# lighttransport/pbrlab

Measured on AMD Instinct MI355X. Metric: Msamples/s (paths x spp / s), 1920x1080 Cornell-box-Suzanne render, higher is better.
Workload: dtype f32

## Files before the change

pbrlab_amd/csrc/bvh_build.cpp:

```cpp
#include <math.h>
#include <stdlib.h>
#include <string.h>

#include <algorithm>
#include <atomic>
#include <deque>
#include <functional>
#include <future>
#include <limits>
#include <thread>

#include "host_scene.h"

namespace pb {
namespace {

#ifndef PB_SAH_BINS
#define PB_SAH_BINS 48
#endif
constexpr int kBins = PB_SAH_BINS;
#ifndef PB_SAH_SWEEP
#define PB_SAH_SWEEP 256
#endif
#ifndef PB_MAX_LEAF_CURVES
// ... 210 lines not shown
    work.push_back({root, 0});
    while (!work.empty()) {
      Item it;
      if (N.size() < (size_t)kTopNodes) it = work.front(), work.pop_front();
      else it = work.back(), work.pop_back();
      const TNode& t = T[it.t];
      depth = std::max(depth, t.depth);
      BvhNode nd;
      memset(&nd, 0, sizeof(nd));
      const TNode &l = T[t.left], &r = T[t.right];
      nd.set_box(0, l.box.lo, l.box.hi);
      nd.set_box(1, r.box.lo, r.box.hi);
      if (l.left < 0) {
        nd.c0 = leaf_ref(l);
      } else {
        nd.c0 = (uint32_t)N.size();
        N.emplace_back();
        work.push_back({t.left, nd.c0});
      }
      if (r.left < 0) {
        nd.c1 = leaf_ref(r);
      } else {
        nd.c1 = (uint32_t)N.size();
        N.emplace_back();
        work.push_back({t.right, nd.c1});
      }
      N[it.out] = nd;
    }
  }
  out->slot_gid = b.order;
  out->depth = depth;
}

struct QBox {
  float lo[3], hi[3];
};
static bool quantise_node(const QBox* c, int n, QNode* nd) {
  memset(nd, 0, sizeof(*nd));
  uint32_t* qw[6] = {&nd->qlo_x, &nd->qlo_y, &nd->qlo_z, &nd->qhi_x, &nd->qhi_y, &nd->qhi_z};
  for (int a = 0; a < 3; a++) {
    float lo = std::numeric_limits<float>::infinity(), hi = -lo;
    for (int i = 0; i < n; i++) lo = std::min(lo, c[i].lo[a]), hi = std::max(hi, c[i].hi[a]);
    if (!(lo <= hi) || !std::isfinite(lo) || !std::isfinite(hi)) return false;
    float sc = std::max(nextafterf((hi - lo) / 253.0f, std::numeric_limits<float>::infinity()), 1.1754944e-38f);
    for (int tries = 0;; tries++) {
      if (tries > 40 || !std::isfinite(sc)) return false;
      const float org = lo;
      bool ok = true;
      uint32_t wl = 0, wh = 0;
      for (int i = 0; i < 4 && ok; i++) {
        if (i >= n) {
          wl |= 255u << (8 * i);
          continue;
        }
        int ql = (int)floor(((double)c[i].lo[a] - (double)org) / (double)sc);
        int qh = (int)ceil(((double)c[i].hi[a] - (double)org) / (double)sc);
        ql = std::max(0, std::min(255, ql)), qh = std::max(0, std::min(255, qh));
        while (ql > 0 && !(fmaf((float)ql, sc, org) <= c[i].lo[a])) ql--;
        while (qh < 255 && !(fmaf((float)qh, sc, org) >= c[i].hi[a])) qh++;
        if (!(fmaf((float)ql, sc, org) <= c[i].lo[a] && fmaf((float)qh, sc, org) >= c[i].hi[a])) ok = false;
        wl |= (uint32_t)ql << (8 * i), wh |= (uint32_t)qh << (8 * i);
      }
      if (ok) {
        nd->org[a] = org;
        (a == 0 ? nd->sx : (a == 1 ? nd->sy : nd->sz)) = sc;
        *qw[a] = wl, *qw[3 + a] = wh;
        break;
      }
      sc *= tries < 8 ? 1.03125f : 2.0f;
    }
  }
  return true;
}

uint32_t build_qtree(const std::vector<BvhNode>& N2, const std::function<uint32_t(uint32_t)>& map_leaf, std::vector<QNode>* out) {
  out->clear();
  if (N2.empty()) return 0;
  struct V {
    float lo[3], hi[3];
    int32_t l = -1, r = -1;
    uint32_t ref = 0;
    uint32_t prims = 0;
  };
  std::vector<V> T;
  T.reserve(N2.size() * 2 + 1);
  {
    struct Todo {
      uint32_t node2;
      int32_t v;
    };
    std::vector<Todo> todo;
    T.emplace_back();
    todo.push_back({0u, 0});
    while (!todo.empty()) {
      const Todo t = todo.back();
      todo.pop_back();
      const BvhNode& b = N2[t.node2];
      int32_t kids[2] = {-1, -1};
      int nk = 0;
      for (int k = 0; k < 2; k++) {
        const uint32_t ref = k ? b.c1 : b.c0;
        if (ref == kEmptyChild) continue;
        const int32_t v = (int32_t)T.size();
        T.emplace_back();
        for (int a = 0; a < 3; a++) T[v].lo[a] = b.lo[a][k], T[v].hi[a] = b.hi[a][k];
        kids[nk++] = v;
        if (ref & kLeafBit) T[v].ref = map_leaf(ref), T[v].prims = (ref & 7u) + 1u;
        else todo.push_back({ref, v});
      }
      if (nk == 2) T[t.v].l = kids[0], T[t.v].r = kids[1];
      else if (nk == 1) T[t.v].l = kids[0], T[t.v].r = -1;
    }
    for (int a = 0; a < 3; a++) {
      T[0].lo[a] = std::numeric_limits<float>::infinity(), T[0].hi[a] = -T[0].lo[a];
      for (int32_t k : {T[0].l, T[0].r})
        if (k >= 0) T[0].lo[a] = std::min(T[0].lo[a], T[k].lo[a]), T[0].hi[a] = std::max(T[0].hi[a], T[k].hi[a]);
    }
  }
  auto area = [](const V& v) {
    const float dx = v.hi[0] - v.lo[0], dy = v.hi[1] - v.lo[1], dz = v.hi[2] - v.lo[2];
    const float a = dx * dy + dy * dz + dz * dx;
    return a >= 0.f && std::isfinite(a) ? (double)a : 0.0;
  };
  constexpr double kCostNode = 1.0, kCostPrim = 1.0;
  const size_t nv = T.size();
  std::vector<double> below(nv, 0.0);
  std::vector<int32_t> choice(nv * 4, -1);
  auto qarea = [&](const V& u, const V& v) {
    double e[3];
    for (int a = 0; a < 3; a++) {
      const double ext = (double)v.hi[a] - (double)v.lo[a];
      const double st = std::max(ext / 253.0, 1e-37);
      const double ql = floor(((double)u.lo[a] - (double)v.lo[a]) / st), qh = ceil(((double)u.hi[a] - (double)v.lo[a]) / st);
      e[a] = std::max(qh - ql, 0.0) * st;
    }
    const double a = e[0] * e[1] + e[1] * e[2] + e[2] * e[0];
    return std::isfinite(a) ? a : 0.0;
  };
  for (size_t vi = nv; vi-- > 0;) {
    const V& v = T[vi];
    if (v.l < 0) continue;
    if (v.r < 0) {
      choice[vi * 4] = v.l;
      below[vi] = T[v.l].l < 0 ? area(T[v.l]) * kCostPrim * T[v.l].prims : area(T[v.l]) * kCostNode + below[v.l];
      continue;
    }
    int32_t fronts[16][4];
    int sizes[16], nf = 0;
    fronts[0][0] = v.l, fronts[0][1] = v.r, sizes[0] = 2, nf = 1;
    for (int i = 0; i < nf && nf < 16; i++) {
      if (sizes[i] >= 4) continue;
      for (int m = 0; m < sizes[i] && nf < 16; m++) {
        const V& u = T[fronts[i][m]];
        if (u.l < 0 || u.r < 0) continue;
        int32_t g[4];
        int n = 0;
        for (int j = 0; j < sizes[i]; j++) {
          if (j == m) g[n++] = u.l, g[n++] = u.r;
          else g[n++] = fronts[i][j];
        }
        std::sort(g, g + n);
        bool dup = false;
        for (int q = 0; q < nf && !dup; q++) dup = sizes[q] == n && std::equal(g, g + n, fronts[q]);
        if (dup) continue;
        std::copy(g, g + n, fronts[nf]), sizes[nf] = n, nf++;
// ... 1 lines not shown
    }
    double best = 1e300;
    int bi = 0;
    for (int i = 0; i < nf; i++) {
      double c = 0.0;
      for (int m = 0; m < sizes[i]; m++) {
        const V& u = T[fronts[i][m]];
        c += u.l < 0 ? qarea(u, v) * kCostPrim * u.prims : qarea(u, v) * kCostNode + below[fronts[i][m]];
      }
      if (c < best) best = c, bi = i;
    }
    below[vi] = best;
    for (int m = 0; m < sizes[bi]; m++) choice[vi * 4 + m] = fronts[bi][m];
  }
  struct Item {
    int32_t v;
    uint32_t out;
  };
  std::deque<Item> work;
  out->emplace_back();
  work.push_back({0, 0u});
  while (!work.empty()) {
    Item it;
    if (out->size() < (size_t)kTopNodes) it = work.front(), work.pop_front();
    else it = work.back(), work.pop_back();
    int32_t fr[4];
    int n = 0;
    if (T[it.v].l < 0) {
      fr[n++] = it.v;
    } else {
      for (int m = 0; m < 4; m++)
        if (choice[(size_t)it.v * 4 + m] >= 0) fr[n++] = choice[(size_t)it.v * 4 + m];
    }
    QBox c[4];
    for (int i = 0; i < n; i++)
      for (int a = 0; a < 3; a++) c[i].lo[a] = T[fr[i]].lo[a], c[i].hi[a] = T[fr[i]].hi[a];
    QNode nd;
    if (n == 0 || !quantise_node(c, n, &nd)) {
      out->clear();
      return 0;
    }
    for (int i = 0; i < 4; i++) nd.c[i] = kEmptyChild;
    for (int i = 0; i < n; i++) {
      const V& u = T[fr[i]];
      if (u.l < 0) {
        nd.c[i] = u.ref;
      } else {
        const uint32_t id = (uint32_t)out->size();
        out->emplace_back();
        nd.c[i] = id;
        work.push_back({fr[i], id});
      }
    }
    (*out)[it.out] = nd;
  }
  std::vector<uint32_t> need(out->size(), 0);
  for (size_t i = out->size(); i-- > 0;) {
    const QNode& nd = (*out)[i];
    uint32_t nc = 0, deepest = 0;
    for (int k = 0; k < 4; k++) {
      if (nd.c[k] == kEmptyChild) continue;
      nc++;
      if (!(nd.c[k] & kLeafBit)) deepest = std::max(deepest, need[nd.c[k]]);
    }
    need[i] = (nc ? nc - 1u : 0u) + deepest;
  }
  return need[0];
}

void build_qlayout(const FlatBvh& bvh, const std::vector<float4>& slots, const std::vector<uint8_t>& kinds, QLayout* out) {
  static_assert(kMaxLeaf <= 2, "a leaf of the binary tree becomes one TriPair / one curve record");
  *out = QLayout();
  std::vector<float4>&qtri = out->tri, &qpts = out->pts;
  std::vector<uint32_t>& qhit = out->hit;
  const float4 zero = make_float4(0.f, 0.f, 0.f, 0.f);
  auto code = [&](uint32_t k) { return k | __builtin_bit_cast(uint32_t, slots[4 * (size_t)k + 2].w); };
  const bool tri_pairs = std::all_of(kinds.begin(), kinds.end(), [](uint8_t kd) { return kd == 0; });
  auto tri_leaf = [&](uint32_t first, uint32_t count) -> uint32_t {
    if (!tri_pairs) {
      const uint32_t rec = (uint32_t)(qtri.size() / 3);
      for (uint32_t i = 0; i < count; i++) {
        for (int c = 0; c < 3; c++) qtri.push_back(slots[4 * (size_t)(first + i) + c]);
        qtri.back().w = __builtin_bit_cast(float, code(first + i));
      }
      return rec;
    }
    const uint32_t rec = (uint32_t)(qtri.size() / kTriPairWords);
    const float4* a = &slots[4 * (size_t)first];
    const float4* b = count == 2 ? &slots[4 * (size_t)(first + 1)] : a;
    const float ca = __builtin_bit_cast(float, code(first)), cb = __builtin_bit_cast(float, count == 2 ? code(first + 1) : kNone);
    qtri.insert(qtri.end(), {make_float4(a[0].x, b[0].x, a[0].y, b[0].y), make_float4(a[0].z, b[0].z, a[1].x, b[1].x),
                             make_float4(a[1].y, b[1].y, a[1].z, b[1].z), make_float4(a[2].x, b[2].x, a[2].y, b[2].y),
                             make_float4(a[2].z, b[2].z, ca, cb)});
    return rec;
  };
  qpts.assign(4, zero);
  qhit.assign(4, kNone);
  auto curve_leaf = [&](uint32_t first, uint32_t count) -> uint32_t {
    while (qpts.size() % 4) qpts.push_back(zero);
    const uint32_t P = (uint32_t)qpts.size();
    uint32_t sub[2] = {0u, 0u};
    for (uint32_t i = 0; i < count; i++) {
      const float4* sl = &slots[4 * (size_t)(first + i)];
      qpts.push_back(sl[0]), qpts.push_back(sl[1]);
      sub[i] = __builtin_bit_cast(uint32_t, sl[2].x) & 3u;
    }
    qhit.resize(qpts.size(), kNone);
    qhit[P] = code(first);
    if (count == 2) qhit[P + 2] = code(first + 1);
    (count == 2 ? out->leaves_pair : out->leaves_one)++;
    return kLeafBit | kCurveBit | ((P | sub[0]) << 3) | (count == 2 ? (kCurvePairBit | sub[1]) : 0u);
  };
  auto map_leaf = [&](uint32_t ref) -> uint32_t {
    const uint32_t first = (ref & 0x3FFFFFFFu) >> 3, count = (ref & 7u) + 1u;
    if (ref & kCurveBit) return curve_leaf(first, count);
    return kLeafBit | (tri_leaf(first, count) << 3) | (count - 1u);
  };
  out->stack_need = build_qtree(bvh.nodes, map_leaf, &out->nodes);
  if (out->stack_need > (uint32_t)kStackDepth || qpts.size() >= (1u << 27)) out->nodes.clear();
  while (qtri.size() % 4) qtri.push_back(zero);
  for (int k = 0; k < 4; k++) qpts.push_back(zero);
  qhit.resize(qpts.size(), kNone);
}

std::vector<SssEntry> build_sss_entries(const std::vector<QNode>& wide, const std::vector<float>& ilo, const std::vector<float>& ihi,
                                        uint32_t max_foreign) {
  const size_t ninst = ilo.size() / 3;
  std::vector<SssEntry> entries(ninst, SssEntry{});
  struct CutRef { uint32_t ref; float lo[3], hi[3]; };
  for (size_t i = 0; i < ninst; i++) {
    SssEntry& E = entries[i];
    if (!(ilo[3 * i] <= ihi[3 * i])) continue;
    float ext = 0.f;
    for (int a = 0; a < 3; a++) ext = std::max(ext, ihi[3 * i + a] - ilo[3 * i + a]);
    if (!(ext > 0.f) || !std::isfinite(ext)) continue;
    const float m1 = 1e-4f * ext, m2 = 2e-3f * ext;
    float rlo[3], rhi[3], wlo[3], whi[3];
    for (int a = 0; a < 3; a++) rlo[a] = ilo[3 * i + a] - m1, rhi[a] = ihi[3 * i + a] + m1, wlo[a] = rlo[a] - m2, whi[a] = rhi[a] + m2;
    std::vector<CutRef> cut{{0u, {-INFINITY, -INFINITY, -INFINITY}, {INFINITY, INFINITY, INFINITY}}};
    for (bool changed = true; changed;) {
      changed = false;
      for (size_t c = 0; c < cut.size() && !changed; c++) {
        if (cut[c].ref & kLeafBit) continue;
        const QNode& nd = wide[cut[c].ref];
        const float org[3] = {nd.org[0], nd.org[1], nd.org[2]}, st3[3] = {nd.sx, nd.sy, nd.sz};
        const uint32_t ql[3] = {nd.qlo_x, nd.qlo_y, nd.qlo_z}, qh[3] = {nd.qhi_x, nd.qhi_y, nd.qhi_z};
        std::vector<CutRef> kids;
        int nchild = 0;
        for (int k = 0; k < 4; k++) {
          if (nd.c[k] == kEmptyChild) continue;
          nchild++;
          CutRef r;
          r.ref = nd.c[k];
          bool meets = true;
          for (int a = 0; a < 3; a++) {
            r.lo[a] = fmaf((float)((ql[a] >> (8 * k)) & 255u), st3[a], org[a]);
            r.hi[a] = fmaf((float)((qh[a] >> (8 * k)) & 255u), st3[a], org[a]);
            meets = meets && r.lo[a] <= whi[a] && r.hi[a] >= wlo[a];
          }
          if (meets) kids.push_back(r);
        }
        if (((int)kids.size() < nchild || kids.size() == 1) && cut.size() - 1 + kids.size() <= 1u + max_foreign) {
          cut.erase(cut.begin() + (ptrdiff_t)c);
          cut.insert(cut.end(), kids.begin(), kids.end());
          changed = true;
        }
      }
    }
    int best = -1;
    double best_v = -1.0;
    for (size_t c = 0; c < cut.size(); c++) {
      if (cut[c].ref & kLeafBit) continue;
      double v = 1.0;
      for (int a = 0; a < 3; a++) v *= std::max(0.0, (double)std::min(cut[c].hi[a], ihi[3 * i + a]) - (double)std::max(cut[c].lo[a], ilo[3 * i + a]));
      if (v > best_v) best_v = v, best = (int)c;
    }
    if (best < 0 || cut[(size_t)best].ref == 0u) continue;
    E.entry = cut[(size_t)best].ref;
// ... 13 lines not shown
```

pbrlab_amd/csrc/dscene.h:

```cpp
#pragma once
#include <math.h>

#include "dclosures.h"

namespace pb {

constexpr uint32_t kLeafBit = 0x80000000u;
constexpr uint32_t kCurveBit = 0x40000000u;
constexpr uint32_t kEmptyChild = 0xFFFFFFFFu;
#ifndef PB_MAX_LEAF
#define PB_MAX_LEAF 2
#endif
constexpr int kMaxLeaf = PB_MAX_LEAF;
#ifndef PB_STACK_DEPTH
#define PB_STACK_DEPTH 64
#endif
constexpr int kStackDepth = PB_STACK_DEPTH;
constexpr int kSimpleLdsStack = 40;
#ifndef PB_TOP_NODES
#define PB_TOP_NODES 64
#endif
constexpr int kTopNodes = PB_TOP_NODES;
#ifndef PB_TOP_NODES_WIDE
#define PB_TOP_NODES_WIDE 0
#endif
constexpr int kTopNodesWide = PB_TOP_NODES_WIDE;

struct alignas(16) BvhNode {
  float lo[3][2];
  float hi[3][2];
  uint32_t c0, c1;
  uint32_t pad[2];
  static float widen_lo(float v) { return v - (fabsf(v) * 1.52587890625e-05f + 1e-30f); }
  static float widen_hi(float v) { return v + (fabsf(v) * 1.52587890625e-05f + 1e-30f); }
  void set_box(int child, const float* l, const float* h) {
    for (int a = 0; a < 3; a++) lo[a][child] = widen_lo(l[a]), hi[a][child] = widen_hi(h[a]);
  }
};
static_assert(sizeof(BvhNode) == 64, "node must be 64 B");

constexpr uint32_t kCurvePairBit = 4u;
struct alignas(16) QNode {
  float org[3], sx;
  float sy, sz;
  uint32_t qlo_x, qlo_y;
  uint32_t qlo_z, qhi_x, qhi_y, qhi_z;
  uint32_t c[4];
};
static_assert(sizeof(QNode) == 64, "quantised wide node must be 64 B");
constexpr uint32_t kTriPairWords = 5;

constexpr uint32_t kQPointHit = 0x80000000u;

constexpr uint32_t kSlotHasNormals = 1u;
constexpr uint32_t kSlotIsCurve = 2u;
constexpr uint32_t kSlotMatHair = 4u;
constexpr uint32_t kSlotMatNone = 8u;
constexpr uint32_t kSlotHasUV = 16u;

struct alignas(128) ShadeRec {
  float ng[3];
  uint32_t matflags;
  float ns_flat[3];
  uint32_t lightrec;
  float n[9];
  uint32_t pad0;
  float uv[6];
  uint32_t gid, instance_id, geom_id, prim_id;
  uint32_t pad[4];
};
static_assert(sizeof(ShadeRec) == 128, "one cache line per primitive");

constexpr uint32_t kHitSlotMask = 0x07FFFFFFu;
constexpr uint32_t kHitMore = 1u << 27;
constexpr uint32_t kHitHair = 1u << 28;
constexpr uint32_t kHitLight = 1u << 29;
constexpr uint32_t kHitNoMaterial = 1u << 30;

struct PrincipledBsdf {
  int enable_diffuse;
// ... 128 lines not shown
```

pbrlab_amd/csrc/dtrace.h:

```cpp
#pragma once

#include "dscene.h"

namespace pb {

struct Hit {
  float t, u, v;
  uint32_t slot;
};

struct TravStats {
  uint32_t nodes, tris, curves;
  uint32_t anodes, atris, acurves;
  uint32_t it_node, it_tri, it_curve, it_refill, ln_node, ln_tri, ln_curve;
  uint32_t hist[8], max_steps;
  uint32_t ahist[8], amax_steps;
  uint32_t refill_ticks;
  unsigned long long cyc[4];
  uint32_t suspended, suspended_any;
  unsigned long long t_exhausted;
};

__device__ __forceinline__ V3 ld3(const float4& a) { return V3(a.x, a.y, a.z); }

// ... 174 lines not shown
  float dist = (ey * pxa - ex * pya) / sqrtf(len2);
  float r = a.w + s * (b.w - a.w);
  if (!(r > 0.0f && fabsf(dist) <= r)) return false;
  float tt = (pza + s * (pzb - pza)) * inv_len;
  if (!(tt > tmin && tt <= tmax)) return false;
  const float rm = __builtin_fmaxf(fabsf(a.w), fabsf(b.w));
  const V3 lo(__builtin_fminf(a.x, b.x) - rm, __builtin_fminf(a.y, b.y) - rm, __builtin_fminf(a.z, b.z) - rm);
  const V3 hi(__builtin_fmaxf(a.x, b.x) + rm, __builtin_fmaxf(a.y, b.y) + rm, __builtin_fmaxf(a.z, b.z) + rm);
  if (!hit_inside(lo, hi, o, inv3, tt)) return false;
  t = tt, u = ((float)i + s) * 0.25f, v = dist / r;
  return true;
}

__device__ __forceinline__ void box_test2(const float4& n0, const float4& n1, const float4& n2, V3 o, V3 inv, float tmin,
                                          float tmax, bool& h0, bool& h1, float& t0, float& t1) {
  const f2 ox = {o.x, o.x}, oy = {o.y, o.y}, oz = {o.z, o.z};
  const f2 ix = {inv.x, inv.x}, iy = {inv.y, inv.y}, iz = {inv.z, inv.z};
  const f2 lx = {n0.x, n0.y}, ly = {n0.z, n0.w}, lz = {n1.x, n1.y};
  const f2 hx = {n1.z, n1.w}, hy = {n2.x, n2.y}, hz = {n2.z, n2.w};
  f2 p = (lx - ox) * ix, q = (hx - ox) * ix;
  f2 a = __builtin_elementwise_min(p, q), b = __builtin_elementwise_max(p, q);
  p = (ly - oy) * iy, q = (hy - oy) * iy;
  a = __builtin_elementwise_max(a, __builtin_elementwise_min(p, q)), b = __builtin_elementwise_min(b, __builtin_elementwise_max(p, q));
  p = (lz - oz) * iz, q = (hz - oz) * iz;
  a = __builtin_elementwise_max(a, __builtin_elementwise_min(p, q)), b = __builtin_elementwise_min(b, __builtin_elementwise_max(p, q));
  const float e = 1.52587890625e-05f;
  const float a0 = __builtin_fmaf(-fabsf(a.x), e, a.x), a1 = __builtin_fmaf(-fabsf(a.y), e, a.y);
  const float b0 = __builtin_fmaf(fabsf(b.x), e, b.x), b1 = __builtin_fmaf(fabsf(b.y), e, b.y);
  t0 = a0, t1 = a1;
  h0 = a0 <= b0 && b0 >= tmin && a0 <= tmax;
  h1 = a1 <= b1 && b1 >= tmin && a1 <= tmax;
}

__device__ __forceinline__ void box_test4q(const float4& w0, const float4& w1, const float4& w2, V3 o, const float4& inv, float ta[4],
                                           float tb[4]) {
  const float e = 1.52587890625e-05f;
  const bool nx = (int)__float_as_uint(inv.x) < 0, ny = (int)__float_as_uint(inv.y) < 0, nz = (int)__float_as_uint(inv.z) < 0;
  const uint32_t qlx = __float_as_uint(w1.z), qly = __float_as_uint(w1.w), qlz = __float_as_uint(w2.x);
  const uint32_t qhx = __float_as_uint(w2.y), qhy = __float_as_uint(w2.z), qhz = __float_as_uint(w2.w);
  const uint32_t lx = nx ? qhx : qlx, ly = ny ? qhy : qly, lz = nz ? qhz : qlz;
  const uint32_t hx = nx ? qlx : qhx, hy = ny ? qly : qhy, hz = nz ? qlz : qhz;
  const f2 sx = {w0.w, w0.w}, sy = {w1.x, w1.x}, sz = {w1.y, w1.y}, gx = {w0.x, w0.x}, gy = {w0.y, w0.y}, gz = {w0.z, w0.z};
  const f2 ox = {o.x, o.x}, oy = {o.y, o.y}, oz = {o.z, o.z}, ix = {inv.x, inv.x}, iy = {inv.y, inv.y}, iz = {inv.z, inv.z};
#pragma unroll
  for (int h = 0; h < 2; h++) {
    auto two = [h](uint32_t w) { return h ? f2{(float)((w >> 16) & 255u), (float)(w >> 24)} : f2{(float)(w & 255u), (float)((w >> 8) & 255u)}; };
    const f2 px = (__builtin_elementwise_fma(two(lx), sx, gx) - ox) * ix, qx = (__builtin_elementwise_fma(two(hx), sx, gx) - ox) * ix;
    const f2 py = (__builtin_elementwise_fma(two(ly), sy, gy) - oy) * iy, qy = (__builtin_elementwise_fma(two(hy), sy, gy) - oy) * iy;
    const f2 pz = (__builtin_elementwise_fma(two(lz), sz, gz) - oz) * iz, qz = (__builtin_elementwise_fma(two(hz), sz, gz) - oz) * iz;
    const float a0 = __builtin_fmaxf(__builtin_fmaxf(px.x, py.x), pz.x), a1 = __builtin_fmaxf(__builtin_fmaxf(px.y, py.y), pz.y);
    const float b0 = __builtin_fminf(__builtin_fminf(qx.x, qy.x), qz.x), b1 = __builtin_fminf(__builtin_fminf(qx.y, qy.y), qz.y);
    ta[2 * h] = __builtin_fmaf(-fabsf(a0), e, a0), ta[2 * h + 1] = __builtin_fmaf(-fabsf(a1), e, a1);
    tb[2 * h] = __builtin_fmaf(fabsf(b0), e, b0), tb[2 * h + 1] = __builtin_fmaf(fabsf(b1), e, b1);
  }
}

constexpr uint32_t kWideMiss = 0xFFFFFFFFu;
__device__ __forceinline__ void wide_node_keys(const float4& w0, const float4& w1, const float4& w2, const float4& refs, V3 o,
                                               const float4& inv, float tmin, float tmax, uint32_t k[4]) {
  float ta[4], tb[4];
  box_test4q(w0, w1, w2, o, inv, ta, tb);
  const uint32_t r[4] = {__float_as_uint(refs.x), __float_as_uint(refs.y), __float_as_uint(refs.z), __float_as_uint(refs.w)};
#pragma unroll
  for (int i = 0; i < 4; i++) {
    const bool h = ta[i] <= tb[i] && tb[i] >= tmin && ta[i] <= tmax && r[i] != kEmptyChild;
    const int bits = (int)__float_as_uint(ta[i]);
    k[i] = h ? ((uint32_t)(bits < 0 ? 0 : bits) & ~3u) | (uint32_t)i : kWideMiss;
  }
  auto cex = [](uint32_t& a, uint32_t& b) {
    const uint32_t lo = a < b ? a : b, hi = a < b ? b : a;
    a = lo, b = hi;
  };
  cex(k[0], k[1]), cex(k[2], k[3]), cex(k[0], k[2]), cex(k[1], k[3]), cex(k[1], k[2]);
}
__device__ __forceinline__ uint32_t wide_ref(const float4& refs, uint32_t key) {
  const uint32_t a = __float_as_uint((key & 1u) ? refs.y : refs.x), b = __float_as_uint((key & 1u) ? refs.w : refs.z);
  return (key & 2u) ? b : a;
}

__device__ __forceinline__ uint32_t q_gid(const DScene& sc, uint32_t code) {
  const uint32_t c = (code & kQPointHit) ? sc.q_hitcode[code & ~kQPointHit] : code;
  return sc.shade[c & kHitSlotMask].gid;
}
__device__ __forceinline__ uint32_t q_final_code(const DScene& sc, uint32_t code) {
  return (code != kNone && (code & kQPointHit)) ? sc.q_hitcode[code & ~kQPointHit] : code;
}

template <int MODE, bool STATS, bool CURVES, bool WIDE = false>
__device__ __forceinline__ bool leaf_test(const DScene& sc, uint32_t leaf, V3 o, V3 d, V3 inv, float tmin, float& best_t,
                                          Hit& hit, TravStats& st, bool any_rt) {
  const bool ANY = MODE == 2 ? any_rt : (MODE == 1);
  uint32_t first = (leaf & 0x3FFFFFFFu) >> 3, count = (leaf & 7u) + 1u;
  bool is_curve = (leaf & kCurveBit) != 0;
  if (WIDE && !CURVES) {
    const float4* g = sc.wide + sc.q_tri0 + (size_t)first * kTriPairWords;
    const float4 w0 = g[0], w1 = g[1], w2 = g[2], w3 = g[3], w4 = g[4];
    uint32_t nt = 0u;
    const bool occluded = tri_pair_accept<MODE == 1, STATS>(sc, w0, w1, w2, w3, w4, o, d, inv, tmin, ANY, hit, nt);
    if (STATS) st.tris += nt;
    best_t = hit.t;
    return occluded;
  }
  const bool rec = WIDE && CURVES && is_curve;
  const uint32_t sub_a = first & 3u, sub_b = leaf & 3u;
  if (rec) first &= ~3u, count = (leaf & kCurvePairBit) ? 2u : 1u;
  for (uint32_t k = 0; k < count; k++) {
    const uint32_t s = first + (rec ? 2u * k : k);
    float t, u, v;
    bool ok;
    uint32_t code;
// ... 29 lines not shown
      const bool less = WIDE ? q_gid(sc, code) < q_gid(sc, hit.slot) : sc.shade[s].gid < sc.shade[hit.slot & kHitSlotMask].gid;
      if (!less) continue;
    }
    best_t = t;
    hit.t = t, hit.u = u, hit.v = v, hit.slot = code;
  }
  return false;
}

template <int MODE, bool STATS, bool CURVES, bool WIDE = false>
__device__ __forceinline__ bool traverse_mode(const DScene& sc, V3 o, V3 d, float tmin, float tmax, Hit& hit,
                                              uint32_t* stack, uint32_t stride, TravStats& st, uint32_t* overflow, bool any_rt,
                                              uint32_t* spill, uint32_t spill_stride) {
  auto push = [&](int& sp, uint32_t v) {
    if (sp < kSimpleLdsStack) stack[(uint32_t)sp * stride] = v, sp++;
    else if (sp < kStackDepth) spill[(uint32_t)(sp - kSimpleLdsStack) * spill_stride] = v, sp++;
    else *overflow = 1u;
  };
  auto pop = [&](int& sp) {
    sp--;
    return sp < kSimpleLdsStack ? stack[(uint32_t)sp * stride] : spill[(uint32_t)(sp - kSimpleLdsStack) * spill_stride];
  };
  hit.slot = kNone;
  hit.t = tmax, hit.u = 0.f, hit.v = 0.f;
  if (sc.num_nodes == 0) return false;
  V3 inv(1.0f / d.x, 1.0f / d.y, 1.0f / d.z);
  float best_t = tmax;
  int sp = 0;
  uint32_t cur = 0;
  for (;;) {
    if (WIDE) {
      const float4* np = sc.wide + (size_t)cur * 4u;
      const float4 w0 = np[0], w1 = np[1], w2 = np[2], refs = np[3];
      if (STATS) st.nodes++;
      uint32_t k[4];
      wide_node_keys(w0, w1, w2, refs, o, make_float4(inv.x, inv.y, inv.z, 0.f), tmin, best_t, k);
#pragma unroll
      for (int j = 3; j >= 1; j--) {
        if (k[j] == kWideMiss) continue;
        push(sp, wide_ref(refs, k[j]));
      }
      uint32_t next = k[0] == kWideMiss ? kEmptyChild : wide_ref(refs, k[0]);
      for (;;) {
        if (next == kEmptyChild) {
          if (sp == 0) {
            hit.slot = q_final_code(sc, hit.slot);
            return hit.slot != kNone;
          }
          next = pop(sp);
        }
        if (!(next & kLeafBit)) break;
        if (leaf_test<MODE, STATS, CURVES, true>(sc, next, o, d, inv, tmin, best_t, hit, st, any_rt)) return true;
        next = kEmptyChild;
      }
      cur = next;
      continue;
    }
    const float4* np = reinterpret_cast<const float4*>(sc.nodes + cur);
    float4 n0 = np[0], n1 = np[1], n2 = np[2], n3 = np[3];
    if (STATS) st.nodes++;
    uint32_t c0 = __float_as_uint(n3.x), c1 = __float_as_uint(n3.y);
    float t0, t1;
    bool h0, h1;
    box_test2(n0, n1, n2, o, inv, tmin, best_t, h0, h1, t0, t1);
    uint32_t next = kEmptyChild;
    if (h0 && h1) {
      uint32_t nearc = c0, farc = c1;
      if (t1 < t0) nearc = c1, farc = c0;
      push(sp, farc);
      next = nearc;
    } else if (h0) {
      next = c0;
    } else if (h1) {
      next = c1;
    }
// ... 21 lines not shown
```

pbrlab_amd/csrc/dtrace_pv.h:

```cpp
#pragma once

#include "dtrace.h"

namespace pb {

#ifndef PB_BATCH
#define PB_BATCH 512
#endif
constexpr uint32_t kPvBatch = PB_BATCH;
#ifndef PB_BATCH_HEADS
#define PB_BATCH_HEADS 256
#endif
constexpr uint32_t kPvBatchHeads = PB_BATCH_HEADS;
constexpr uint32_t kPvHeadStride = 64;
#ifndef PB_GUIDE
#define PB_GUIDE 2
#endif
constexpr uint32_t kPvGuide = PB_GUIDE;
#ifndef PB_LDS_STACK
#define PB_LDS_STACK 16
#endif
constexpr int kPvLdsStack = PB_LDS_STACK;
#ifndef PB_LDS_STACK_DEEP
#define PB_LDS_STACK_DEEP 20
#endif
constexpr int kPvLdsStackDeep = PB_LDS_STACK_DEEP;
template <bool CURVES, bool WIDE>
__host__ __device__ constexpr int pv_lds_stack() { return (CURVES && WIDE) ? kPvLdsStackDeep : kPvLdsStack; }
#ifndef PB_REFILL
#define PB_REFILL 32
#endif
constexpr int kPvRefillIdle = PB_REFILL;
#ifndef PB_REFILL_CURVES
#define PB_REFILL_CURVES 24
#endif
constexpr int kPvRefillIdleCurves = PB_REFILL_CURVES;
#ifndef PB_WALK_REFILL
#define PB_WALK_REFILL 56
#endif
#ifndef PB_W_NODE
#define PB_W_NODE 1
#endif
#ifndef PB_W_TRI
#define PB_W_TRI 2
#endif
#ifndef PB_W_CURVE
#define PB_W_CURVE 2
#endif

enum : uint32_t { kStIdle = 0, kStNode = 1, kStTri = 2, kStCurve = 3, kStDone = 4, kStDoneOccluded = 5 };

template <typename Sink, typename = void>
struct SinkSplits { static constexpr bool value = false; };
template <typename Sink>
struct SinkSplits<Sink, decltype((void)Sink::kSplit)> { static constexpr bool value = Sink::kSplit && !Sink::kWalk; };
template <typename Sink>
__device__ constexpr bool sink_splits() { return SinkSplits<Sink>::value; }
template <typename Sink, typename = void>
struct SinkSuspends { static constexpr bool value = false; };
template <typename Sink>
struct SinkSuspends<Sink, decltype((void)Sink::kSuspend)> { static constexpr bool value = Sink::kSuspend && !Sink::kWalk; };
template <typename Sink>
__device__ constexpr bool sink_suspends() { return SinkSuspends<Sink>::value; }
constexpr uint32_t kTagShadow = 0x80000000u, kTagNoSuspend = 0x40000000u, kTagResume = 0x20000000u, kTagHeld = 0x10000000u;
constexpr uint32_t kSuspRecWords = 72;

template <int MODE, bool STATS, bool CURVES, bool WIDE, uint32_t NHEADS = 1u, typename Sink>
__device__ __forceinline__ void trace_pv(const DScene& sc, uint32_t n, uint32_t* head, Sink& sink, uint32_t* stk_base,
                                         uint32_t stride, uint32_t* spill, uint32_t spill_stride, TravStats& st,
                                         uint32_t* overflow, float* frame = nullptr, const float4* top = nullptr,
                                         uint32_t ntop = 0) {
  constexpr uint32_t nheads = NHEADS;
  constexpr int kLds = pv_lds_stack<CURVES, WIDE>();
  const uint32_t lane = __lane_id();
  auto rank_in = [](unsigned long long m) {
    return (uint32_t)__builtin_amdgcn_mbcnt_hi((uint32_t)(m >> 32), __builtin_amdgcn_mbcnt_lo((uint32_t)m, 0u));
  };
  uint32_t batch_cur = 0, batch_end = 0;
  const uint32_t waves_total = gridDim.x * (blockDim.x >> 6);
  uint32_t hsel = nheads > 1u ? blockIdx.x % nheads : 0u, heads_left = nheads;
  const uint32_t kBatchCap = nheads > 1u ? kPvBatchHeads : kPvBatch;
  uint32_t batch = n / waves_total;
  if (batch >= 64u) {
    batch = (kPvGuide ? n / (waves_total * kPvGuide) : batch) & ~63u;
    batch = batch > kBatchCap ? kBatchCap : (batch < 64u ? 64u : batch);
  } else {
    batch = (n + waves_total - 1u) / waves_total;
    batch = batch < 1u ? 1u : batch;
  }
  bool exhausted = (n == 0) || (sc.num_nodes == 0);
  if (sc.num_nodes == 0 && n != 0) {
    for (;;) {
      uint32_t base = 0;
      if (lane == 0) base = atomicAdd(head, 64u);
      base = (uint32_t)__shfl((int)base, 0);
      if (base >= n) break;
      uint32_t idx = base + lane;
      if (idx < n) {
        uint32_t tag;
        V3 o, d;
        float tmin, tmax;
        sink.load(idx, tag, o, d, tmin, tmax);
        Hit h = {tmax, 0.f, 0.f, kNone};
        sink.done(tag, h, false);
      }
    }
// ... 174 lines not shown
      }
      unsigned long long node_mask = __ballot(state == kStNode);
      unsigned long long tri_mask = __ballot(state == kStTri);
      int n_node = __popcll(node_mask), n_tri = __popcll(tri_mask);
      int n_curve = CURVES ? __popcll(__ballot(state == kStCurve)) : 0;
      const int w_node = n_node * PB_W_NODE, w_tri = n_tri * PB_W_TRI, w_curve = n_curve * PB_W_CURVE;
      const int phase = (w_node >= w_tri && w_node >= w_curve) ? 0 : ((!CURVES || w_tri >= w_curve) ? 1 : 2);
      did = phase;
      if (STATS && lane == 0) {
        if (phase == 0) st.it_node++, st.ln_node += n_node;
        else if (phase == 1) st.it_tri++, st.ln_tri += n_tri;
        else st.it_curve++, st.ln_curve += n_curve;
      }
      if (phase == 0) {
        if (WIDE && state == kStNode) {
          if (STATS) (any_ray ? st.anodes : st.nodes)++, steps++;
#ifdef PB_DIAG_EXTRA_VALU
          {
            float x = D0.x;
#pragma unroll
            for (int k2 = 0; k2 < PB_DIAG_EXTRA_VALU; k2++) asm volatile("v_fma_f32 %0, %0, %0, %1" : "+v"(x) : "v"(D0.y));
            if (x == 1.2345e-30f) tmin = x;
          }
#endif
#ifdef PB_DIAG_EXTRA_LOAD
          {
            const float4* qd = items + cur;
            asm volatile("" : "+v"(qd));
            const float4 x = *qd;
            if (x.x == 1.2345e-30f) tmin = x.y;
          }
#endif
          uint32_t k[4];
          wide_node_keys(D0, D1, D2, D3w, o, inv4, tmin, hit.t, k);
          auto ref_of = [&](uint32_t key) { return wide_ref(D3w, key); };
          advance = true;
          have_next = k[0] != kWideMiss;
          next = ref_of(k[0]);
          if (!CURVES && k[1] != kWideMiss) {
            if (sp + 3 <= kLds) {
              uint32_t p = (uint32_t)sp;
              stk_base[p * stride] = ref_of(k[3]);
              p += (k[3] != kWideMiss) ? 1u : 0u;
              stk_base[p * stride] = ref_of(k[2]);
              p += (k[2] != kWideMiss) ? 1u : 0u;
              stk_base[p * stride] = ref_of(k[1]);
              sp = (int)p + 1;
            } else {
#pragma unroll
              for (int j = 3; j >= 1; j--) {
                if (k[j] == kWideMiss) continue;
                const uint32_t farc = ref_of(k[j]);
                if (sp < kLds) {
                  stk_base[(uint32_t)sp * stride] = farc;
                  sp++;
                } else if (sp < kStackDepth) {
                  spill[(uint32_t)(sp - kLds) * spill_stride] = farc;
                  sp++;
                } else {
                  *overflow = 1u;
                }
              }
            }
          } else if (k[1] != kWideMiss) {
            const uint32_t r3 = ref_of(k[3]), r2 = ref_of(k[2]), r1 = ref_of(k[1]);
            const uint32_t p3 = (uint32_t)sp, p2 = p3 + ((k[3] != kWideMiss) ? 1u : 0u), p1 = p2 + ((k[2] != kWideMiss) ? 1u : 0u);
            if (__ballot(p1 >= (uint32_t)kLds) == 0ull) {
              stk_base[p3 * stride] = r3;
// ... 119 lines not shown
      if (!have_next) {
        if (sp == 0) {
          state = kStDone;
          advance = false;
          if (STATS) {
            const int b = steps <= 16u ? 0 : (28 - __clz(steps - 1u) > 7 ? 7 : 28 - __clz(steps - 1u));
            if (any_ray) st.ahist[b]++, st.amax_steps = steps > st.amax_steps ? steps : st.amax_steps;
            else st.hist[b]++, st.max_steps = steps > st.max_steps ? steps : st.max_steps;
          }
        } else {
          sp--;
          next = stk_base[(uint32_t)(sp < kLds ? sp : kLds - 1) * stride];
          if (sp >= kLds) next = spill[(uint32_t)(sp - kLds) * spill_stride];
        }
      }
      if (advance) {
        need_load = true;
        if (next & kLeafBit) {
          const uint32_t first = (next & 0x3FFFFFFFu) >> 3;
          rem = next & 7u;
          state = (CURVES && (next & kCurveBit)) ? kStCurve : kStTri;
          if (WIDE && !CURVES) rem = 0u;
          if (WIDE) cur = (CURVES && (next & kCurveBit)) ? sc.q_pt0 + first : sc.q_tri0 + (CURVES ? 3u : kTriPairWords) * first;
          else cur = first + slot0;
        } else {
          cur = WIDE ? 4u * next : next;
          state = kStNode;
        }
      }
    }
    if (WIDE && need_load) {
      if (!CURVES && kTopNodesWide > 0 && cur < 4u * ntop) {
        const float4* g = top + cur;
        D0 = g[0], D1 = g[1], D2 = g[2], D3w = g[3];
      } else {
        const bool at_rec = CURVES && state == kStCurve;
        const float4* g = items + (at_rec ? (cur & ~3u) : cur);
        D0 = g[0], D1 = g[1];
        if (!CURVES || state != kStCurve || at_rec) D2 = g[2];
        if (!CURVES || state == kStNode || at_rec) D3w = g[3];
        if (!CURVES && state == kStTri) D4 = g[4];
      }
    } else if (need_load) {
      if (kTopNodes > 0 && cur < ntop) {
        const float4* g = top + cur * 4u;
        D0 = g[0], D1 = g[1], D2 = g[2];
        D3 = *reinterpret_cast<const float2*>(g + 3);
      } else {
        const float4* g = reinterpret_cast<const float4*>(sc.nodes + cur);
        D0 = g[0], D1 = g[1], D2 = g[2];
        if (state == kStNode) D3 = *reinterpret_cast<const float2*>(g + 3);
      }
    }
  }
  if constexpr (!Sink::kWalk) {
    if (state >= kStDone) {
      if (WIDE && CURVES) hit.slot = q_final_code(sc, hit.slot);
      sink.done(tag, hit, state == kStDoneOccluded);
    }
  }
  if constexpr (sink_suspends<Sink>()) {
    if (state >= kStNode && state <= kStCurve) {
      const uint32_t j = wave_id * 64u + __lane_id();
      uint32_t* rec = sink.susp_out() + (size_t)j * kSuspRecWords;
      rec[0] = __float_as_uint(hit.t), rec[1] = __float_as_uint(hit.u), rec[2] = __float_as_uint(hit.v), rec[3] = hit.slot;
      rec[4] = cur, rec[5] = state | (rem << 8) | ((uint32_t)sp << 16);
      for (int i = 0; i < sp; i++) rec[8 + i] = i < kLds ? stk_base[(uint32_t)i * stride] : spill[(uint32_t)(i - kLds) * spill_stride];
      sink.suspended(tag, j, o, d);
      if (STATS) (any_ray ? st.suspended_any : st.suspended)++;
    }
  }
}

// ... 2 lines not shown
```

pbrlab_amd/csrc/dtrace_quad.h:

```cpp
#pragma once

#include "dtrace.h"

namespace pb {

template <int CTRL>
__device__ __forceinline__ uint32_t quad_perm(uint32_t v) {
  return (uint32_t)__builtin_amdgcn_mov_dpp((int)v, CTRL, 0xF, 0xF, true);
}
constexpr int kQp1032 = 0xB1, kQp2301 = 0x4E, kQp1230 = 0x39, kQp3012 = 0x93;
__device__ __forceinline__ uint32_t quad_min_u32(uint32_t v) {
  uint32_t w = quad_perm<kQp1032>(v);
  v = v < w ? v : w;
  w = quad_perm<kQp2301>(v);
  return v < w ? v : w;
}
__device__ __forceinline__ float quad_from(float v, uint32_t src_lane) { return __shfl(v, (int)src_lane); }
__device__ __forceinline__ uint32_t quad_from(uint32_t v, uint32_t src_lane) { return (uint32_t)__shfl((int)v, (int)src_lane); }
__device__ __forceinline__ float4 quad_from(const float4& v, uint32_t src_lane) {
  return make_float4(quad_from(v.x, src_lane), quad_from(v.y, src_lane), quad_from(v.z, src_lane), quad_from(v.w, src_lane));
}

__device__ __forceinline__ void box_test1q(const float4& w0, const float4& w1, const float4& w2, uint32_t j, V3 o, V3 inv, float& ta, float& tb) {
  const float e = 1.52587890625e-05f;
  const uint32_t sh = 8u * j;
  auto q = [sh](float w) { return (float)((__float_as_uint(w) >> sh) & 255u); };
  float p = (__builtin_fmaf(q(w1.z), w0.w, w0.x) - o.x) * inv.x, r = (__builtin_fmaf(q(w2.y), w0.w, w0.x) - o.x) * inv.x;
  float a = __builtin_fminf(p, r), b = __builtin_fmaxf(p, r);
  p = (__builtin_fmaf(q(w1.w), w1.x, w0.y) - o.y) * inv.y, r = (__builtin_fmaf(q(w2.z), w1.x, w0.y) - o.y) * inv.y;
  a = __builtin_fmaxf(a, __builtin_fminf(p, r)), b = __builtin_fminf(b, __builtin_fmaxf(p, r));
  p = (__builtin_fmaf(q(w2.x), w1.y, w0.z) - o.z) * inv.z, r = (__builtin_fmaf(q(w2.w), w1.y, w0.z) - o.z) * inv.z;
  a = __builtin_fmaxf(a, __builtin_fminf(p, r)), b = __builtin_fminf(b, __builtin_fmaxf(p, r));
  ta = __builtin_fmaf(-fabsf(a), e, a), tb = __builtin_fmaf(fabsf(b), e, b);
}

template <int MODE>
__device__ __forceinline__ bool traverse_quad(const DScene& sc, V3 o, V3 d, float tmin, float tmax, Hit& hit, uint32_t* stack, uint32_t stride,
                                              uint32_t* overflow, bool any_rt, uint32_t* spill, uint32_t spill_stride) {
  const bool any_ray = MODE == 2 ? any_rt : (MODE == 1);
  hit.slot = kNone, hit.t = tmax, hit.u = 0.f, hit.v = 0.f;
  if (sc.num_nodes == 0) return false;
  const uint32_t lane = __lane_id(), j = lane & 3u, qbase = lane & ~3u;
  const V3 inv(1.0f / d.x, 1.0f / d.y, 1.0f / d.z);
  const float4* const items = sc.wide;
  auto put = [&](uint32_t pos, uint32_t ref) {
    if (pos < (uint32_t)kSimpleLdsStack) stack[pos * stride] = ref;
    else if (pos < (uint32_t)kStackDepth) spill[(pos - (uint32_t)kSimpleLdsStack) * spill_stride] = ref;
    else *overflow = 1u;
  };
  auto get = [&](uint32_t pos) { return pos < (uint32_t)kSimpleLdsStack ? stack[pos * stride] : spill[(pos - (uint32_t)kSimpleLdsStack) * spill_stride]; };
  uint32_t sp = 0u, next = 0u;
  uint32_t holder = 4u;
  float4 P0 = make_float4(0.f, 0.f, 0.f, 0.f), P1 = P0, P2 = P0, P3 = P0, P4 = P0;
  bool occluded = false;
  for (;;) {
    float4 N0, N1, N2, N3;
    if (holder < 4u) {
      N0 = quad_from(P0, qbase + holder), N1 = quad_from(P1, qbase + holder), N2 = quad_from(P2, qbase + holder), N3 = quad_from(P3, qbase + holder);
    } else {
      const float4* g = items + 4u * next;
      N0 = g[0], N1 = g[1], N2 = g[2], N3 = g[3];
    }
    const uint32_t ref = __float_as_uint(j == 0u ? N3.x : (j == 1u ? N3.y : (j == 2u ? N3.z : N3.w)));
    if (ref != kEmptyChild) {
// ... 56 lines not shown
```

Baseline: 2950.

## Pack quantised node steps as exponents and derive child refs from base offsets

Quantisation steps in each wide BVH node become power-of-two exponents packed into one word, alongside child counts. Inner children are laid out contiguously and leaf triangle records are repacked per node, so child references can be computed from two base words. The traversal in the persistent/wide path can then skip loading the fourth 16-byte word (explicit refs) of each node, and the box test is split into near-side and far-side passes to ease register pressure. Power-of-two steps make the quantised boxes slightly looser, which may add some extra box hits, and the leaf repacking changes memory locality.

```diff
diff --git a/pbrlab_amd/csrc/bvh_build.cpp b/pbrlab_amd/csrc/bvh_build.cpp
--- a/pbrlab_amd/csrc/bvh_build.cpp
+++ b/pbrlab_amd/csrc/bvh_build.cpp
@@ -266,6 +266,15 @@
   out->depth = depth;
 }
 
+static uint32_t qstep_exponent(float extent) {
+  const float x = nextafterf(extent / 253.0f, std::numeric_limits<float>::infinity());
+  if (!std::isfinite(x) || !(x >= 0.f)) return 0u;
+  const uint32_t bits = __builtin_bit_cast(uint32_t, x);
+  const uint32_t e = std::max((bits >> 23) + ((bits & 0x7FFFFFu) ? 1u : 0u), 1u);
+  return e <= 254u ? e : 0u;
+}
+static float qstep(uint32_t e) { return __builtin_bit_cast(float, e << 23); }
+
 struct QBox {
   float lo[3], hi[3];
 };
@@ -276,10 +285,10 @@
     float lo = std::numeric_limits<float>::infinity(), hi = -lo;
     for (int i = 0; i < n; i++) lo = std::min(lo, c[i].lo[a]), hi = std::max(hi, c[i].hi[a]);
     if (!(lo <= hi) || !std::isfinite(lo) || !std::isfinite(hi)) return false;
-    float sc = std::max(nextafterf((hi - lo) / 253.0f, std::numeric_limits<float>::infinity()), 1.1754944e-38f);
-    for (int tries = 0;; tries++) {
-      if (tries > 40 || !std::isfinite(sc)) return false;
-      const float org = lo;
+    uint32_t e = qstep_exponent(hi - lo);
+    for (;; e++) {
+      if (e == 0u || e > 254u) return false;
+      const float sc = qstep(e), org = lo;
       bool ok = true;
       uint32_t wl = 0, wh = 0;
       for (int i = 0; i < 4 && ok; i++) {
@@ -297,11 +306,10 @@
       }
       if (ok) {
         nd->org[a] = org;
-        (a == 0 ? nd->sx : (a == 1 ? nd->sy : nd->sz)) = sc;
+        nd->pack |= e << (8 * a);
         *qw[a] = wl, *qw[3 + a] = wh;
         break;
       }
-      sc *= tries < 8 ? 1.03125f : 2.0f;
     }
   }
   return true;
@@ -364,7 +372,8 @@
     double e[3];
     for (int a = 0; a < 3; a++) {
       const double ext = (double)v.hi[a] - (double)v.lo[a];
-      const double st = std::max(ext / 253.0, 1e-37);
+      const uint32_t se = qstep_exponent((float)ext);
+      const double st = se ? (double)qstep(se) : std::max(ext / 253.0, 1e-37);
       const double ql = floor(((double)u.lo[a] - (double)v.lo[a]) / st), qh = ceil(((double)u.hi[a] - (double)v.lo[a]) / st);
       e[a] = std::max(qh - ql, 0.0) * st;
     }
@@ -432,6 +441,7 @@
       for (int m = 0; m < 4; m++)
         if (choice[(size_t)it.v * 4 + m] >= 0) fr[n++] = choice[(size_t)it.v * 4 + m];
     }
+    std::stable_partition(fr, fr + n, [&](int32_t u) { return T[u].l >= 0; });
     QBox c[4];
     for (int i = 0; i < n; i++)
       for (int a = 0; a < 3; a++) c[i].lo[a] = T[fr[i]].lo[a], c[i].hi[a] = T[fr[i]].hi[a];
@@ -441,6 +451,8 @@
       return 0;
     }
     for (int i = 0; i < 4; i++) nd.c[i] = kEmptyChild;
+    uint32_t n_inner = 0;
+    nd.inner_base = (uint32_t)out->size();
     for (int i = 0; i < n; i++) {
       const V& u = T[fr[i]];
       if (u.l < 0) {
@@ -449,9 +461,12 @@
         const uint32_t id = (uint32_t)out->size();
         out->emplace_back();
         nd.c[i] = id;
+        n_inner++;
         work.push_back({fr[i], id});
       }
     }
+    nd.pack |= n_inner << 24 | (uint32_t)n << 28;
+    nd.leaf_word = 0u;
     (*out)[it.out] = nd;
   }
   std::vector<uint32_t> need(out->size(), 0);
@@ -518,6 +533,20 @@
   };
   out->stack_need = build_qtree(bvh.nodes, map_leaf, &out->nodes);
   if (out->stack_need > (uint32_t)kStackDepth || qpts.size() >= (1u << 27)) out->nodes.clear();
+  if (tri_pairs) {
+    std::vector<float4> packed;
+    packed.reserve(qtri.size());
+    for (QNode& nd : out->nodes) {
+      const uint32_t ni = nd.n_inner(), nc = nd.n_children(), base = (uint32_t)(packed.size() / kTriPairWords);
+      for (uint32_t i = ni; i < nc; i++) {
+        const uint32_t rec = (nd.c[i] & 0x3FFFFFFFu) >> 3;
+        packed.insert(packed.end(), qtri.begin() + (size_t)rec * kTriPairWords, qtri.begin() + (size_t)(rec + 1u) * kTriPairWords);
+        nd.c[i] = kLeafBit | ((base + i - ni) << 3) | (nd.c[i] & 7u);
+      }
+      nd.leaf_word = kLeafBit + ((base - ni) << 3);
+    }
+    if (!out->nodes.empty()) qtri.swap(packed);
+  }
   while (qtri.size() % 4) qtri.push_back(zero);
   for (int k = 0; k < 4; k++) qpts.push_back(zero);
   qhit.resize(qpts.size(), kNone);
@@ -543,7 +572,7 @@
       for (size_t c = 0; c < cut.size() && !changed; c++) {
         if (cut[c].ref & kLeafBit) continue;
         const QNode& nd = wide[cut[c].ref];
-        const float org[3] = {nd.org[0], nd.org[1], nd.org[2]}, st3[3] = {nd.sx, nd.sy, nd.sz};
+        const float org[3] = {nd.org[0], nd.org[1], nd.org[2]}, st3[3] = {nd.step(0), nd.step(1), nd.step(2)};
         const uint32_t ql[3] = {nd.qlo_x, nd.qlo_y, nd.qlo_z}, qh[3] = {nd.qhi_x, nd.qhi_y, nd.qhi_z};
         std::vector<CutRef> kids;
         int nchild = 0;
diff --git a/pbrlab_amd/csrc/dscene.h b/pbrlab_amd/csrc/dscene.h
--- a/pbrlab_amd/csrc/dscene.h
+++ b/pbrlab_amd/csrc/dscene.h
@@ -41,11 +41,15 @@
 
 constexpr uint32_t kCurvePairBit = 4u;
 struct alignas(16) QNode {
-  float org[3], sx;
-  float sy, sz;
-  uint32_t qlo_x, qlo_y;
-  uint32_t qlo_z, qhi_x, qhi_y, qhi_z;
+  float org[3];
+  uint32_t pack;
+  uint32_t qlo_x, qlo_y, qlo_z, qhi_x;
+  uint32_t qhi_y, qhi_z, inner_base, leaf_word;
   uint32_t c[4];
+  PB_HD float step(int axis) const { return __builtin_bit_cast(float, ((pack >> (8 * axis)) & 255u) << 23); }
+  PB_HD uint32_t n_inner() const { return (pack >> 24) & 15u; }
+  PB_HD uint32_t n_children() const { return pack >> 28; }
+  PB_HD uint32_t derived_ref(uint32_t i) const { return i < n_inner() ? inner_base + i : leaf_word + (i << 3); }
 };
 static_assert(sizeof(QNode) == 64, "quantised wide node must be 64 B");
 constexpr uint32_t kTriPairWords = 5;
diff --git a/pbrlab_amd/csrc/dtrace.h b/pbrlab_amd/csrc/dtrace.h
--- a/pbrlab_amd/csrc/dtrace.h
+++ b/pbrlab_amd/csrc/dtrace.h
@@ -230,38 +230,72 @@
   h1 = a1 <= b1 && b1 >= tmin && a1 <= tmax;
 }
 
+template <int AXIS>
+__device__ __forceinline__ float qnode_step(const float4& w0) {
+  return __uint_as_float((__float_as_uint(w0.w) << (23 - 8 * AXIS)) & 0x7F800000u);
+}
+template <bool SIDES = false>
 __device__ __forceinline__ void box_test4q(const float4& w0, const float4& w1, const float4& w2, V3 o, const float4& inv, float ta[4],
                                            float tb[4]) {
   const float e = 1.52587890625e-05f;
   const bool nx = (int)__float_as_uint(inv.x) < 0, ny = (int)__float_as_uint(inv.y) < 0, nz = (int)__float_as_uint(inv.z) < 0;
-  const uint32_t qlx = __float_as_uint(w1.z), qly = __float_as_uint(w1.w), qlz = __float_as_uint(w2.x);
-  const uint32_t qhx = __float_as_uint(w2.y), qhy = __float_as_uint(w2.z), qhz = __float_as_uint(w2.w);
-  const uint32_t lx = nx ? qhx : qlx, ly = ny ? qhy : qly, lz = nz ? qhz : qlz;
-  const uint32_t hx = nx ? qlx : qhx, hy = ny ? qly : qhy, hz = nz ? qlz : qhz;
-  const f2 sx = {w0.w, w0.w}, sy = {w1.x, w1.x}, sz = {w1.y, w1.y}, gx = {w0.x, w0.x}, gy = {w0.y, w0.y}, gz = {w0.z, w0.z};
+  const uint32_t qlx = __float_as_uint(w1.x), qly = __float_as_uint(w1.y), qlz = __float_as_uint(w1.z);
+  const uint32_t qhx = __float_as_uint(w1.w), qhy = __float_as_uint(w2.x), qhz = __float_as_uint(w2.y);
+  const float s0 = qnode_step<0>(w0), s1 = qnode_step<1>(w0), s2 = qnode_step<2>(w0);
+  const f2 sx = {s0, s0}, sy = {s1, s1}, sz = {s2, s2}, gx = {w0.x, w0.x}, gy = {w0.y, w0.y}, gz = {w0.z, w0.z};
   const f2 ox = {o.x, o.x}, oy = {o.y, o.y}, oz = {o.z, o.z}, ix = {inv.x, inv.x}, iy = {inv.y, inv.y}, iz = {inv.z, inv.z};
+  auto lo2 = [](uint32_t w) { return f2{(float)(w & 255u), (float)((w >> 8) & 255u)}; };
+  auto hi2 = [](uint32_t w) { return f2{(float)((w >> 16) & 255u), (float)(w >> 24)}; };
+  if (SIDES) {
+    {
+      const uint32_t lx = nx ? qhx : qlx, ly = ny ? qhy : qly, lz = nz ? qhz : qlz;
 #pragma unroll
-  for (int h = 0; h < 2; h++) {
-    auto two = [h](uint32_t w) { return h ? f2{(float)((w >> 16) & 255u), (float)(w >> 24)} : f2{(float)(w & 255u), (float)((w >> 8) & 255u)}; };
-    const f2 px = (__builtin_elementwise_fma(two(lx), sx, gx) - ox) * ix, qx = (__builtin_elementwise_fma(two(hx), sx, gx) - ox) * ix;
-    const f2 py = (__builtin_elementwise_fma(two(ly), sy, gy) - oy) * iy, qy = (__builtin_elementwise_fma(two(hy), sy, gy) - oy) * iy;
-    const f2 pz = (__builtin_elementwise_fma(two(lz), sz, gz) - oz) * iz, qz = (__builtin_elementwise_fma(two(hz), sz, gz) - oz) * iz;
-    const float a0 = __builtin_fmaxf(__builtin_fmaxf(px.x, py.x), pz.x), a1 = __builtin_fmaxf(__builtin_fmaxf(px.y, py.y), pz.y);
-    const float b0 = __builtin_fminf(__builtin_fminf(qx.x, qy.x), qz.x), b1 = __builtin_fminf(__builtin_fminf(qx.y, qy.y), qz.y);
-    ta[2 * h] = __builtin_fmaf(-fabsf(a0), e, a0), ta[2 * h + 1] = __builtin_fmaf(-fabsf(a1), e, a1);
-    tb[2 * h] = __builtin_fmaf(fabsf(b0), e, b0), tb[2 * h + 1] = __builtin_fmaf(fabsf(b1), e, b1);
+      for (int h = 0; h < 2; h++) {
+        const f2 px = (__builtin_elementwise_fma(h ? hi2(lx) : lo2(lx), sx, gx) - ox) * ix;
+        const f2 py = (__builtin_elementwise_fma(h ? hi2(ly) : lo2(ly), sy, gy) - oy) * iy;
+        const f2 pz = (__builtin_elementwise_fma(h ? hi2(lz) : lo2(lz), sz, gz) - oz) * iz;
+        const float a0 = __builtin_fmaxf(__builtin_fmaxf(px.x, py.x), pz.x), a1 = __builtin_fmaxf(__builtin_fmaxf(px.y, py.y), pz.y);
+        ta[2 * h] = __builtin_fmaf(-fabsf(a0), e, a0), ta[2 * h + 1] = __builtin_fmaf(-fabsf(a1), e, a1);
+      }
+    }
+    {
+      const uint32_t hx = nx ? qlx : qhx, hy = ny ? qly : qhy, hz = nz ? qlz : qhz;
+#pragma unroll
+      for (int h = 0; h < 2; h++) {
+        const f2 qx = (__builtin_elementwise_fma(h ? hi2(hx) : lo2(hx), sx, gx) - ox) * ix;
+        const f2 qy = (__builtin_elementwise_fma(h ? hi2(hy) : lo2(hy), sy, gy) - oy) * iy;
+        const f2 qz = (__builtin_elementwise_fma(h ? hi2(hz) : lo2(hz), sz, gz) - oz) * iz;
+        const float b0 = __builtin_fminf(__builtin_fminf(qx.x, qy.x), qz.x), b1 = __builtin_fminf(__builtin_fminf(qx.y, qy.y), qz.y);
+        tb[2 * h] = __builtin_fmaf(fabsf(b0), e, b0), tb[2 * h + 1] = __builtin_fmaf(fabsf(b1), e, b1);
+      }
+    }
+  } else {
+    const uint32_t lx = nx ? qhx : qlx, ly = ny ? qhy : qly, lz = nz ? qhz : qlz;
+    const uint32_t hx = nx ? qlx : qhx, hy = ny ? qly : qhy, hz = nz ? qlz : qhz;
+#pragma unroll
+    for (int h = 0; h < 2; h++) {
+      auto two = [&](uint32_t w) { return h ? hi2(w) : lo2(w); };
+      const f2 px = (__builtin_elementwise_fma(two(lx), sx, gx) - ox) * ix, qx = (__builtin_elementwise_fma(two(hx), sx, gx) - ox) * ix;
+      const f2 py = (__builtin_elementwise_fma(two(ly), sy, gy) - oy) * iy, qy = (__builtin_elementwise_fma(two(hy), sy, gy) - oy) * iy;
+      const f2 pz = (__builtin_elementwise_fma(two(lz), sz, gz) - oz) * iz, qz = (__builtin_elementwise_fma(two(hz), sz, gz) - oz) * iz;
+      const float a0 = __builtin_fmaxf(__builtin_fmaxf(px.x, py.x), pz.x), a1 = __builtin_fmaxf(__builtin_fmaxf(px.y, py.y), pz.y);
+      const float b0 = __builtin_fminf(__builtin_fminf(qx.x, qy.x), qz.x), b1 = __builtin_fminf(__builtin_fminf(qx.y, qy.y), qz.y);
+      ta[2 * h] = __builtin_fmaf(-fabsf(a0), e, a0), ta[2 * h + 1] = __builtin_fmaf(-fabsf(a1), e, a1);
+      tb[2 * h] = __builtin_fmaf(fabsf(b0), e, b0), tb[2 * h + 1] = __builtin_fmaf(fabsf(b1), e, b1);
+    }
   }
 }
 
 constexpr uint32_t kWideMiss = 0xFFFFFFFFu;
-__device__ __forceinline__ void wide_node_keys(const float4& w0, const float4& w1, const float4& w2, const float4& refs, V3 o,
+template <bool SIDES = false>
+__device__ __forceinline__ void wide_node_keys(const float4& w0, const float4& w1, const float4& w2, V3 o,
                                                const float4& inv, float tmin, float tmax, uint32_t k[4]) {
   float ta[4], tb[4];
-  box_test4q(w0, w1, w2, o, inv, ta, tb);
-  const uint32_t r[4] = {__float_as_uint(refs.x), __float_as_uint(refs.y), __float_as_uint(refs.z), __float_as_uint(refs.w)};
+  box_test4q<SIDES>(w0, w1, w2, o, inv, ta, tb);
+  const uint32_t nch = __float_as_uint(w0.w) >> 28;
 #pragma unroll
   for (int i = 0; i < 4; i++) {
-    const bool h = ta[i] <= tb[i] && tb[i] >= tmin && ta[i] <= tmax && r[i] != kEmptyChild;
+    const bool h = ta[i] <= tb[i] && tb[i] >= tmin && ta[i] <= tmax && (uint32_t)i < nch;
     const int bits = (int)__float_as_uint(ta[i]);
     k[i] = h ? ((uint32_t)(bits < 0 ? 0 : bits) & ~3u) | (uint32_t)i : kWideMiss;
   }
@@ -274,6 +308,10 @@
 __device__ __forceinline__ uint32_t wide_ref(const float4& refs, uint32_t key) {
   const uint32_t a = __float_as_uint((key & 1u) ? refs.y : refs.x), b = __float_as_uint((key & 1u) ? refs.w : refs.z);
   return (key & 2u) ? b : a;
+}
+__device__ __forceinline__ uint32_t wide_ref_derived(const float4& w0, const float4& w2, uint32_t key) {
+  const uint32_t i = key & 3u, n_inner = (__float_as_uint(w0.w) >> 24) & 15u;
+  return i < n_inner ? __float_as_uint(w2.z) + i : __float_as_uint(w2.w) + (i << 3);
 }
 
 __device__ __forceinline__ uint32_t q_gid(const DScene& sc, uint32_t code) {
@@ -369,15 +407,16 @@
     if (WIDE) {
       const float4* np = sc.wide + (size_t)cur * 4u;
       const float4 w0 = np[0], w1 = np[1], w2 = np[2], refs = np[3];
+      auto ref_of = [&](uint32_t key) { return wide_ref(refs, key); };
       if (STATS) st.nodes++;
       uint32_t k[4];
-      wide_node_keys(w0, w1, w2, refs, o, make_float4(inv.x, inv.y, inv.z, 0.f), tmin, best_t, k);
+      wide_node_keys(w0, w1, w2, o, make_float4(inv.x, inv.y, inv.z, 0.f), tmin, best_t, k);
 #pragma unroll
       for (int j = 3; j >= 1; j--) {
         if (k[j] == kWideMiss) continue;
-        push(sp, wide_ref(refs, k[j]));
-      }
-      uint32_t next = k[0] == kWideMiss ? kEmptyChild : wide_ref(refs, k[0]);
+        push(sp, ref_of(k[j]));
+      }
+      uint32_t next = k[0] == kWideMiss ? kEmptyChild : ref_of(k[0]);
       for (;;) {
         if (next == kEmptyChild) {
           if (sp == 0) {
diff --git a/pbrlab_amd/csrc/dtrace_pv.h b/pbrlab_amd/csrc/dtrace_pv.h
--- a/pbrlab_amd/csrc/dtrace_pv.h
+++ b/pbrlab_amd/csrc/dtrace_pv.h
@@ -37,6 +37,9 @@
 constexpr int kPvRefillIdleCurves = PB_REFILL_CURVES;
 #ifndef PB_WALK_REFILL
 #define PB_WALK_REFILL 56
+#endif
+#ifndef PB_QNODE_LOAD_REFS
+#define PB_QNODE_LOAD_REFS 0
 #endif
 #ifndef PB_W_NODE
 #define PB_W_NODE 1
@@ -72,6 +75,7 @@
                                          uint32_t ntop = 0) {
   constexpr uint32_t nheads = NHEADS;
   constexpr int kLds = pv_lds_stack<CURVES, WIDE>();
+  constexpr bool kLoadRefs = CURVES || PB_QNODE_LOAD_REFS != 0;
   const uint32_t lane = __lane_id();
   auto rank_in = [](unsigned long long m) {
     return (uint32_t)__builtin_amdgcn_mbcnt_hi((uint32_t)(m >> 32), __builtin_amdgcn_mbcnt_lo((uint32_t)m, 0u));
@@ -312,8 +316,8 @@
           }
 #endif
           uint32_t k[4];
-          wide_node_keys(D0, D1, D2, D3w, o, inv4, tmin, hit.t, k);
-          auto ref_of = [&](uint32_t key) { return wide_ref(D3w, key); };
+          wide_node_keys<true>(D0, D1, D2, o, inv4, tmin, hit.t, k);
+          auto ref_of = [&](uint32_t key) { return kLoadRefs ? wide_ref(D3w, key) : wide_ref_derived(D0, D2, key); };
           advance = true;
           have_next = k[0] != kWideMiss;
           next = ref_of(k[0]);
@@ -499,13 +503,14 @@
     if (WIDE && need_load) {
       if (!CURVES && kTopNodesWide > 0 && cur < 4u * ntop) {
         const float4* g = top + cur;
-        D0 = g[0], D1 = g[1], D2 = g[2], D3w = g[3];
+        D0 = g[0], D1 = g[1], D2 = g[2];
+        if (kLoadRefs) D3w = g[3];
       } else {
         const bool at_rec = CURVES && state == kStCurve;
         const float4* g = items + (at_rec ? (cur & ~3u) : cur);
         D0 = g[0], D1 = g[1];
         if (!CURVES || state != kStCurve || at_rec) D2 = g[2];
-        if (!CURVES || state == kStNode || at_rec) D3w = g[3];
+        if (CURVES ? (state == kStNode || at_rec) : (kLoadRefs || state == kStTri)) D3w = g[3];
         if (!CURVES && state == kStTri) D4 = g[4];
       }
     } else if (need_load) {
diff --git a/pbrlab_amd/csrc/dtrace_quad.h b/pbrlab_amd/csrc/dtrace_quad.h
--- a/pbrlab_amd/csrc/dtrace_quad.h
+++ b/pbrlab_amd/csrc/dtrace_quad.h
@@ -25,11 +25,12 @@
   const float e = 1.52587890625e-05f;
   const uint32_t sh = 8u * j;
   auto q = [sh](float w) { return (float)((__float_as_uint(w) >> sh) & 255u); };
-  float p = (__builtin_fmaf(q(w1.z), w0.w, w0.x) - o.x) * inv.x, r = (__builtin_fmaf(q(w2.y), w0.w, w0.x) - o.x) * inv.x;
+  const float sx = qnode_step<0>(w0), sy = qnode_step<1>(w0), sz = qnode_step<2>(w0);
+  float p = (__builtin_fmaf(q(w1.x), sx, w0.x) - o.x) * inv.x, r = (__builtin_fmaf(q(w1.w), sx, w0.x) - o.x) * inv.x;
   float a = __builtin_fminf(p, r), b = __builtin_fmaxf(p, r);
-  p = (__builtin_fmaf(q(w1.w), w1.x, w0.y) - o.y) * inv.y, r = (__builtin_fmaf(q(w2.z), w1.x, w0.y) - o.y) * inv.y;
+  p = (__builtin_fmaf(q(w1.y), sy, w0.y) - o.y) * inv.y, r = (__builtin_fmaf(q(w2.x), sy, w0.y) - o.y) * inv.y;
   a = __builtin_fmaxf(a, __builtin_fminf(p, r)), b = __builtin_fminf(b, __builtin_fmaxf(p, r));
-  p = (__builtin_fmaf(q(w2.x), w1.y, w0.z) - o.z) * inv.z, r = (__builtin_fmaf(q(w2.w), w1.y, w0.z) - o.z) * inv.z;
+  p = (__builtin_fmaf(q(w1.z), sz, w0.z) - o.z) * inv.z, r = (__builtin_fmaf(q(w2.y), sz, w0.z) - o.z) * inv.z;
   a = __builtin_fmaxf(a, __builtin_fminf(p, r)), b = __builtin_fminf(b, __builtin_fmaxf(p, r));
   ta = __builtin_fmaf(-fabsf(a), e, a), tb = __builtin_fmaf(fabsf(b), e, b);
 }
```

Result: no change. 2940 (-0.4%).
